# BiaPyX/BiaPy

Hardware: AMD Instinct MI355X
Metric: voxels/sec 3D ResUNet 128^3 patch (train: fwd+bwd+AdamW; sub-records: infer, sliding) (higher is better)
Workload: dtype f16 forward/activations + bf16 gradients (MFMA f16 / bf16, fp32 accumulate)

## Files before the change

biapy_amd/_lib.py:

```python
from __future__ import annotations

import ctypes as C
import os
from typing import Optional

import torch

_HERE = os.path.dirname(os.path.abspath(__file__))
LIB_PATH = os.environ.get("BPX_LIB_PATH") or os.path.join(_HERE, "libbiapy_amd.so")

F32, BF16, F16, U8, MIX16 = 0, 1, 2, 3, 4
ACT = {"none": 0, "linear": 0, "elu": 1, "relu": 2, "silu": 3, "leaky_relu": 4, "gelu": 5, "tanh": 6, "sigmoid": 7, "softplus": 8}
PK_K3, PK_K3_T, PK_K1, PK_DENSE, PK_DENSE_T, PK_CT, PK_CT_T, PK_CT4, PK_CT4_T = range(9)


class AxisGrid(C.Structure):
    _fields_ = [("n", C.c_int32), ("step", C.c_int32), ("last", C.c_int32), ("patch", C.c_int32), ("limit", C.c_int32)]


class Tensor(C.Structure):
    _fields_ = [("ptr", C.c_void_p), ("ld", C.c_int32), ("C", C.c_int32), ("cs", C.c_int64)]


NULL_T = Tensor(None, 0, 0, 0)
# ... 41 lines not shown
    "bpx_seg_loss_blocks": ([_i64], _i),
    "bpx_seg_loss_sums": ([_vp, _vp, _i64, _vp, _vp], _i),
    "bpx_seg_loss_bwd": ([_vp, _vp, _i64, _vp, _vp, _vp], _i),
    "bpx_seg_loss_finish": ([_vp, _i, _i64, _f, _f, _f, _vp, _vp, _vp], _i),
    "bpx_seg_loss_bwd_fused": ([_vp, _vp, _i64, _vp, _vp, _f, _f, _f, _vp, _vp], _i),
    "bpx_softmax_ce_blocks": ([_i64], _i),
    "bpx_softmax_ce_row": ([], _i),
    "bpx_softmax_ce_sums": ([_vp, _vp, _i, _i, _i64, _i, _vp, _vp, _vp], _i),
    "bpx_softmax_ce_finish": ([_vp, _i, _i64, _vp, _vp, _vp], _i),
    "bpx_softmax_ce_bwd": ([_vp, _vp, _i, _i, _i64, _i, _vp, _vp, _vp, _vp, _vp], _i),
    "bpx_dice_blocks": ([_i64], _i),
    "bpx_dice_row": ([], _i),
    "bpx_dice_sums": ([_vp, _vp, _i, _i, _i64, _i, _i, _vp, _i, _vp, _vp], _i),
    "bpx_dice_finish": ([_vp, _i, _i, _i64, _i, _i, C.c_double, C.c_double, C.c_double, _vp, _vp, _vp, _vp], _i),
    "bpx_dice_bwd": ([_vp, _vp, _i, _i, _i64, _i, _i, _i, _vp, _vp, _vp, _vp, _vp], _i),
    "bpx_chan_loss_finish": ([_vp, _i, _i, _i64, _vp, _vp, _vp], _i),
    "bpx_chan_loss_bwd_fused": ([_vp, _vp, _i, _i, _i64, C.c_uint, _vp, _vp, _vp, _vp], _i),
    "bpx_conv3d_fwd": ([_i, _i, _i, _i, _i, Tensor, _vp, _i, _vp, _vp, Tensor, _vp, _vp, Tensor, _vp, _vp], _i),
    "bpx_conv3d_fwd_pool": ([_i, _i, _i, _i, _i, Tensor, _vp, _i, _vp, _vp, Tensor, _vp, _vp, Tensor, _vp, _i, Tensor, _vp, _vp], _i),
    "bpx_conv3d_fwd_pool_supported": ([_i, _i, _i, _i, _i, _i, _i, _i], _i),
    "bpx_conv3d_fwd_shuffle": ([_i, _i, _i, _i, _i, Tensor, _vp, _i, _vp, _vp, _i, Tensor, _vp], _i),
    "bpx_conv3d_stats_tiles": ([_i, _i, _i, _i, _i, _i], _i),
    "bpx_conv3d_dgrad": ([_i, _i, _i, _i, _i, Tensor, _vp, Tensor, _vp, _i, Tensor, _vp, _vp], _i),
    "bpx_conv3d_wgrad": ([_i, _i, _i, _i, _i, Tensor, _vp, _i, Tensor, _i, _vp, _vp, _vp, _i64, _vp], _i),
    "bpx_conv3d_wgrad_db2": ([_i, _i, _i, _i, _i, Tensor, _vp, _i, Tensor, _i, _vp, _vp, _vp, _vp, _i64, _vp], _i),
    "bpx_conv3d_wgrad_workspace": ([_i, _i, _i, _i, _i, _i, _i], _i64),
    "bpx_conv3d_bwd_fused_supported": ([_i, _i, _i, _i, _i, _i, _i], _i),
    "bpx_conv3d_bwd_fused_stats_tiles": ([_i, _i, _i, _i, _i, _i], _i),
    "bpx_conv3d_bwd_fused_workspace": ([_i, _i, _i, _i, _i, _i], _i64),
    "bpx_conv3d_bwd_fused": ([_i, _i, _i, _i, _i, Tensor, _vp, Tensor, _vp, _i, Tensor, _vp, _vp, _vp, _vp, _vp, _i64, _vp], _i),
    "bpx_debug_set_bwd_fused": ([_i], _i),
    "bpx_debug_set_bwd_rs": ([_i], _i),
    "bpx_debug_set_conv_kg": ([_i], _i),
    "bpx_debug_set_tile_order": ([_i], _i),
    "bpx_debug_set_wgrad_cap": ([_i], _i),
    "bpx_debug_set_wgrad_k1": ([_i], _i),
    "bpx_debug_set_pw_stream": ([_i], _i),
    "bpx_debug_set_convt_k1": ([_i], _i),
    "bpx_debug_set_c1_persist": ([_i], _i),
    "bpx_convT3d_k2s2_wgrad_workspace": ([_i, _i, _i, _i, _i, _i, _i], _i64),
    "bpx_conv1x1_fwd": ([_i, _i, _i64, Tensor, _vp, _vp, Tensor, Tensor, _vp, Tensor, Tensor, _vp], _i),
    "bpx_conv1x1_fwd_split_wgrad_workspace": ([_i, _i, _i64, _i], _i64),
    "bpx_conv1x1_fwd_split_wgrad_query": ([_i, _i, _i64, Tensor, Tensor, Tensor, _vp, Tensor, Tensor], _i64),
    "bpx_conv1x1_fwd_split_wgrad": ([_i, _i, _i64, Tensor, _vp, Tensor, Tensor, _vp, Tensor, Tensor, _vp, _vp, _i64, _vp], _i),
    "bpx_conv1x1_fwd_split": ([_i, _i, _i64, Tensor, _vp, _vp, Tensor, Tensor, _vp, Tensor, Tensor, Tensor, _vp], _i),
    "bpx_convT3d_k2s2_fwd": ([_i, _i, _i, _i, _i, _i, Tensor, _vp, _vp, Tensor, _vp, _vp], _i),
    "bpx_convT3d_stats_tiles": ([_i, _i, _i, _i], _i),
    "bpx_convT3d_k2s2_dgrad": ([_i, _i, _i, _i, _i, _i, Tensor, _vp, Tensor, _vp], _i),
    "bpx_convT3d_k2s2_wgrad": ([_i, _i, _i, _i, _i, _i, Tensor, Tensor, _vp, _vp, _vp, _i64, _vp], _i),
    "bpx_convT3d_k2s2_bwd": ([_i, _i, _i, _i, _i, _i, Tensor, Tensor, _vp, Tensor, _vp, _vp, _vp, _i64, _vp], _i),
    "bpx_debug_set_convt_bwd": ([_i], _i),
    "bpx_debug_convt_bwd_launches": ([], _i),
    "bpx_norm_finalize": ([_vp, _i, _i, _i, _i64, _vp, _vp, _f, _i, _vp, _i, _i, _vp], _i),
    "bpx_norm_channel_sums": ([_vp, _i, _i, _i, _vp, _i, _i, _vp], _i),
    "bpx_groupnorm_finalize": ([_vp, _i, _i, _i64, _vp, _vp, _f, _i, _vp, _vp], _i),
    "bpx_groupnorm_bwd_finalize": ([_vp, _i, _i, _i64, _vp, _vp, _vp, _vp, _i, _vp, _vp], _i),
    "bpx_tensor_stats": ([_i, _i, _i64, Tensor, _vp, _vp], _i),
    "bpx_tensor_stats_tiles": ([_i64], _i),
    "bpx_norm_bwd_finalize": ([_vp, _i, _i, _i, _i64, _vp, _vp, _vp, _vp, _i, _vp, _vp], _i),
    "bpx_norm_bwd_finalize_deferred": ([_vp, _i, _i, _i, _i64, _vp, _vp, _vp, _vp, _i, _vp, _vp], _i),
    "bpx_batchnorm_finalize": ([_vp, _i, _i, _i, _i64, _vp, _vp, _f, _f, _vp, _vp, _vp, _vp, _i, _i, _vp], _i),
    "bpx_batchnorm_bwd_finalize": ([_vp, _i, _i, _i, _i64, _vp, _vp, _vp, _vp, _i, _vp, _vp], _i),
    "bpx_batchnorm_eval_records": ([_i, _vp, _i, _vp], _i),
    "bpx_gather3d_tables": ([_vp, _i, _i, _i, _i, _i, _vp, _i, _i, _i, _i, _vp, _vp], _i),
    "bpx_scatter3d_tables": ([_vp, _i, _vp, _i, _i, _i, _i, _vp, _i, _i, _i, _i, _vp], _i),
    "bpx_scatter3d_regions": ([_vp, _i, _i, _i, _i, _i, _vp, _vp, _i, _i, _i, _vp], _i),
# ... 202 lines not shown
```

biapy_amd/csrc/conv3d_igemm.hip:

```cpp
#include "conv3d_shared.h"

using namespace bpxconv;

namespace bpxconv { long long* g_conv_stamps = nullptr; }
#define g_stamps bpxconv::g_conv_stamps
extern "C" int bpx_debug_set_conv_stamps(void* p) { g_stamps = (long long*)p; return 0; }
static int g_use_ws = 0;
static int g_conv_kg = -1;
extern "C" int bpx_debug_set_conv_kg(int on) { g_conv_kg = on; return 0; }
static int64_t g_lean_min_vps = 32768;

namespace {

template <typename T, int EZ, int EY, int EX>
__device__ __forceinline__ void stage_block(unsigned char* smem, const T* __restrict__ src, int ld, int cs, int chunk, int n, int D, int H,
                                            int W, int oz, int oy, int ox, const bpx_norm_rec* __restrict__ norm, int C_norm,
                                            int act, int tid) {
  constexpr int KPL = ElemTraits<T>::KPL, GPT = 16 / KPL, VB = 16 * (int)sizeof(T);
  constexpr int PIECES = EZ * EY * EX * GPT;
  constexpr int UNR = 4;
  const int sub = tid % GPT;
  float sc[KPL], sh[KPL];
  if (norm) {
#pragma unroll
    for (int e = 0; e < KPL; ++e) {
      bpx_norm_rec r = norm[(size_t)n * C_norm + chunk * 16 + sub * KPL + e];
      sc[e] = r.scale; sh[e] = r.shift;
    }
  }
  const T* sbase = src + (size_t)chunk * cs + sub * KPL;
  for (int base = 0; base < PIECES; base += 256 * UNR) {
    u32x4_t buf[UNR];
    bool ok[UNR];
#pragma unroll
    for (int u = 0; u < UNR; ++u) {
      int idx = base + u * 256 + tid;
      ok[u] = false;
      buf[u] = u32x4_t{0u, 0u, 0u, 0u};
      if (idx < PIECES) {
        int hv = idx / GPT;
        int hx = hv % EX, hy = (hv / EX) % EY, hz = hv / (EX * EY);
        int gz = oz + hz, gy = oy + hy, gx = ox + hx;
// ... 1 lines not shown
          ok[u] = true;
          buf[u] = *reinterpret_cast<const u32x4_t*>(sbase + ((((size_t)n * D + gz) * H + gy) * W + gx) * (size_t)ld);
        }
      }
    }
#pragma unroll
    for (int u = 0; u < UNR; ++u) {
      int idx = base + u * 256 + tid;
      if (idx < PIECES) {
        u32x4_t v = buf[u];
        if (norm && ok[u]) {
          float f[KPL];
          unpack16<T>(v, f);
#pragma unroll
          for (int e = 0; e < KPL; ++e) f[e] = fmaf(sc[e], f[e], sh[e]);
          bpx_act_vec<std::is_same<T, float>::value, KPL>(f, act);
          v = pack16<T>(f);
        }
        *reinterpret_cast<u32x4_t*>(smem + (size_t)(idx / GPT) * VB + sub * 16) = v;
      }
    }
  }
}

__host__ __device__ constexpr int wreg_next(int s, int np, int per) {
  int k = 0;
  for (int t = np; t < s; ++t) {
    int c = t + 1 - k;
    k += c < per ? (c > 0 ? c : 0) : per;
  }
  return k;
}

template <typename T, int TZ, int TY, int TX, int NS, int EPI, int ACTK, typename TT = T, int KG = 1>
__global__ void __launch_bounds__(256 * KG, 2) conv3_kernel(const Conv3Params p) {
  using Tr = ElemTraits<T>;
  constexpr int KPL = Tr::KPL, GPT = 16 / KPL, VB = 16 * (int)sizeof(T);
  constexpr int HZ = TZ + 2, HY = TY + 2, HX = TX + 2, HV = HZ * HY * HX;
  constexpr int QTOT = 27 * GPT, STEPS = (QTOT + 3) / 4, QPAD = STEPS * 4;
  constexpr int MT = TZ * TY * TX / 16, MS = MT / 4;
  static_assert(MT % 4 == 0 && MS >= 1, "tile must give every wave at least one m-subtile");
  static_assert((HV * GPT + 255) / 256 <= STEPS, "one staged piece per MFMA step");
  static_assert(sizeof(T) != 2 || wreg_next(STEPS, (HV * GPT + 255) / 256, (STEPS + (STEPS - (HV * GPT + 255) / 256) - 1) / (STEPS - (HV * GPT + 255) / 256)) == STEPS, "weight re-load schedule must cover every fragment");
  constexpr int RED_BYTES = 4 * NS * 16 * 2 * 4;
  constexpr int BUFB = HV * VB;
  static_assert(NS * 16 * 2 * 4 * 4 <= RED_BYTES, "reduction scratch");
  constexpr int NBUF = 2;
  static_assert(KG == 1 || (TX == 8 && sizeof(T) == 2), "two K groups: the small-tile 16-bit instances only");
  constexpr int XCH_BYTES = KG == 2 ? MS * NS * 256 * 16 : 0;
  static_assert(XCH_BYTES <= KG * NBUF * BUFB, "accumulator exchange fits the halo buffers");
  __shared__ __attribute__((aligned(16))) unsigned char smem_all[KG * NBUF * BUFB + RED_BYTES];

  const int kg = KG == 2 ? __builtin_amdgcn_readfirstlane((int)(threadIdx.x >> 8)) : 0;
  unsigned char* const smem = smem_all + kg * NBUF * BUFB;
  const int tid = threadIdx.x & 255, lane = tid & 63, wave = tid >> 6;
  const int j = lane & 15, g = lane >> 4;
  const int tile = blockIdx.x % p.tilesPerSample, n = blockIdx.x / p.tilesPerSample;
  const int txi = tile % p.tilesX, tyi = (tile / p.tilesX) % p.tilesY, tzi = tile / (p.tilesX * p.tilesY);
  const int z0 = tzi * TZ, y0 = tyi * TY, x0 = txi * TX;
  const int co_base = blockIdx.y * 16 * NS;
  const int Cout = p.Cout;

  int stamp_i = 0;
#define BPX_STAMP() do { if (p.stamps && tid == 0 && kg == 0 && blockIdx.y == 0 && stamp_i < 15) p.stamps[(size_t)blockIdx.x * 16 + stamp_i++] = (long long)__builtin_readcyclecounter(); } while (0)
  BPX_STAMP();
  if (p.stamps && tid == 0 && kg == 0 && blockIdx.y == 0)
    p.stamps[(size_t)blockIdx.x * 16 + 15] =
        (long long)(((unsigned long long)__builtin_amdgcn_s_getreg((31 << 11) | 20) << 32) | (unsigned)__builtin_amdgcn_s_getreg((31 << 11) | 4));
  f32x4_t acc[MS][NS];
#pragma unroll
  for (int ms = 0; ms < MS; ++ms)
#pragma unroll
    for (int ns = 0; ns < NS; ++ns) acc[ms][ns] = f32x4_t{0.f, 0.f, 0.f, 0.f};

  static_assert(TZ == 4 && MS * 16 == TY * TX && (TX == 16 || TX == 8), "wave = z-slice mapping");
  constexpr int HSTR = (TX >= 16 ? 1 : 16 / TX) * HX * VB;
  constexpr int TSTR = 16 * VB;
  int hb0, tb0;
  {
    int t = (wave * MS) * 16 + j;
    int tz = t / (TY * TX), ty = (t / TX) % TY, tx = t % TX;
    hb0 = ((tz * HY + ty) * HX + tx) * VB;
    tb0 = t * VB;
  }
  const int cg_off = (GPT == 2 ? (g & 1) : g) * 16;
  const bool hi_tap = (GPT == 2) && (g >> 1);
  constexpr int NCLS = (GPT == 2) ? 4 : 1;
  int lbase[NCLS];
  if (GPT == 2) {
    lbase[0] = hb0 + cg_off + (hi_tap ? VB : 0);
    lbase[1 % NCLS] = hb0 + cg_off + (hi_tap ? HX * VB : 0);
    lbase[2 % NCLS] = hb0 + cg_off + (hi_tap ? HY * HX * VB : 0);
    lbase[NCLS - 1] = hb0 + cg_off;
  } else {
    lbase[0] = hb0 + cg_off;
  }

  constexpr int NPIECE = HV * GPT;
  constexpr int NP = (NPIECE + 255) / 256;
  const int sub = tid % GPT;
  uint32_t goff[NP];
#pragma unroll
  for (int u = 0; u < NP; ++u) {
    int idx = u * 256 + tid;
    goff[u] = 0xFFFFFFFFu;
    if (idx < NPIECE) {
      int hv = idx / GPT;
      int hx = hv % HX, hy = (hv / HX) % HY, hz = hv / (HX * HY);
      int gz = z0 - 1 + hz, gy = y0 - 1 + hy, gx = x0 - 1 + hx;
      if (gz >= 0 && gz < p.D && gy >= 0 && gy < p.H && gx >= 0 && gx < p.W)
        goff[u] = (uint32_t)((((uint32_t)gz * p.H + gy) * p.W + gx) * (uint32_t)p.x_ld);
    }
  }
  const T* __restrict__ xin = reinterpret_cast<const T*>(p.x) + (size_t)n * p.D * p.H * p.W * p.x_ld + sub * KPL;
  const T* __restrict__ wp = reinterpret_cast<const T*>(p.wp);
  const bpx_norm_rec* __restrict__ nrec = p.in_norm ? p.in_norm + (size_t)n * p.Cin + sub * KPL : nullptr;
  const int nchunks = p.Cin / 16;

  u32x4_t pbuf[NP];
  float psc[KPL], psh[KPL];

#define BPX_STAGE_PIECE(u, wbuf, next_chunk)                                                                  \
  do {                                                                                                        \
    const int idx_ = (u) * 256 + tid;                                                                         \
    if (idx_ < NPIECE) {                                                                                      \
      u32x4_t v_ = pbuf[u];                                                                                   \
      if (nrec && goff[u] != 0xFFFFFFFFu && !(p.dbg & 2)) {                                                   \
        float f_[KPL];                                                                                        \
        unpack16<T>(v_, f_);                                                                                  \
        if (ACTK == 1) { _Pragma("unroll") for (int e_ = 0; e_ < KPL; ++e_) f_[e_] = apply_act_rt<T, 1>(fmaf(psc[e_], f_[e_], psh[e_]), p.act); } \
        else { _Pragma("unroll") for (int e_ = 0; e_ < KPL; ++e_) f_[e_] = fmaf(psc[e_], f_[e_], psh[e_]);                    \
               bpx_act_vec<std::is_same<T, float>::value, KPL, ACTK == 2>(f_, p.act); }                                               \
        v_ = pack16<T>(f_);                                                                                   \
      }                                                                                                       \
      *reinterpret_cast<u32x4_t*>(smem + (wbuf) + (size_t)idx_ * 16) = v_;                                    \
      if ((next_chunk) < nchunks && goff[u] != 0xFFFFFFFFu && !(p.dbg & 4))                                   \
        pbuf[u] = *reinterpret_cast<const u32x4_t*>(xin + goff[u] + (size_t)(next_chunk) * p.x_cs);                       \
    }                                                                                                         \
  } while (0)
#define BPX_LOAD_NORM(chunk_)                                                                                 \
  do {                                                                                                        \
    if (nrec && (chunk_) < nchunks) {                                                                         \
      _Pragma("unroll") for (int e_ = 0; e_ < KPL; ++e_) {                                                    \
        bpx_norm_rec r_ = nrec[(chunk_) * 16 + e_];                                                           \
        psc[e_] = r_.scale; psh[e_] = r_.shift;                                                               \
      }                                                                                                       \
    }                                                                                                         \
  } while (0)

  BPX_STAMP();
  {
#pragma unroll
  for (int u = 0; u < NP; ++u) {
    pbuf[u] = u32x4_t{0u, 0u, 0u, 0u};
    if (goff[u] != 0xFFFFFFFFu) pbuf[u] = *reinterpret_cast<const u32x4_t*>(xin + goff[u] + (size_t)kg * p.x_cs);
  }
  BPX_LOAD_NORM(kg);
#pragma unroll
  for (int u = 0; u < NP; ++u) BPX_STAGE_PIECE(u, 0, kg + KG);
  BPX_LOAD_NORM(kg + KG);
  BPX_STAMP();
  __syncthreads();
  BPX_STAMP();

  constexpr bool WREG = (sizeof(T) == 2) && (STEPS * NS * 4 <= 112);
  constexpr int NWR = WREG ? STEPS : 1;
  constexpr int WSTEPS = STEPS - NP;
  constexpr int PER = WREG ? (STEPS + WSTEPS - 1) / WSTEPS : 1;
  u32x4_t wreg[NWR][NS];
  if (WREG) {
    const T* wl0 = wp + ((size_t)kg * QPAD * Cout + (size_t)g * Cout + co_base + j) * KPL;
#pragma unroll
    for (int s = 0; s < NWR; ++s)
#pragma unroll
      for (int ns = 0; ns < NS; ++ns) wreg[s][ns] = *reinterpret_cast<const u32x4_t*>(wl0 + ((size_t)s * 4 * Cout + ns * 16) * KPL);
  }
  constexpr bool SMALL = TX == 8;
  constexpr int WD = SMALL ? 3 : 1;
  constexpr int NAF = SMALL ? 2 : 1;
  u32x4_t wq[WREG ? 1 : WD + 1][NS];
  if (!WREG) {
    const T* wl0 = wp + ((size_t)kg * QPAD * Cout + (size_t)g * Cout + co_base + j) * KPL;
#pragma unroll
    for (int d = 0; d < WD; ++d)
#pragma unroll
      for (int ns = 0; ns < NS; ++ns) wq[d][ns] = *reinterpret_cast<const u32x4_t*>(wl0 + ((size_t)d * 4 * Cout + ns * 16) * KPL);
  }
  int cur = 0;
  for (int chunk = kg; chunk < nchunks; chunk += KG) {
    const int nxt = BUFB - cur;
    const bool stage_next = chunk + KG < nchunks;
    const T* wl = wp + ((size_t)chunk * QPAD * Cout + (size_t)g * Cout + co_base + j) * KPL;
    const T* wl1 = wl + (size_t)KG * QPAD * Cout * KPL;
    u32x4_t af[NAF][MS];
    auto read_frags = [&](int s_, u32x4_t* f) {
      const int tapA = (GPT == 2) ? bpx_tap_order_bf16(2 * s_) : s_;
      const int cls = (GPT == 2) ? (s_ < 9 ? 0 : s_ < 12 ? 1 : s_ == 12 ? 2 : 3) : 0;
      const int imm = tap_off<HY, HX, VB>(tapA);
#pragma unroll
      for (int ms = 0; ms < MS; ++ms) f[ms] = *reinterpret_cast<const u32x4_t*>(smem + lbase[cls] + ms * HSTR + imm);
    };
    if (NAF == 2) read_frags(0, af[0]);
#pragma unroll
    for (int s = 0; s < STEPS; ++s) {
      if (!WREG && s + WD < STEPS) {
#pragma unroll
        for (int ns = 0; ns < NS; ++ns)
          wq[WREG ? 0 : (s + WD) % (WD + 1)][ns] = *reinterpret_cast<const u32x4_t*>(wl + ((size_t)(s + WD) * 4 * Cout + ns * 16) * KPL);
      }
      if (NAF == 2) { if (s + 1 < STEPS) read_frags(s + 1, af[(s + 1) % NAF]); }
      else read_frags(s, af[0]);
      __builtin_amdgcn_sched_barrier(0);
#pragma unroll
      for (int ms = 0; ms < MS; ++ms) {
#pragma unroll
        for (int ns = 0; ns < NS; ++ns) acc[ms][ns] = mfma_step<T>(WREG ? wreg[WREG ? s : 0][ns] : wq[WREG ? 0 : s % (WD + 1)][ns], af[s % NAF][ms], acc[ms][ns]);
      }
      if (s < NP && stage_next) BPX_STAGE_PIECE(s < NP ? s : 0, nxt, chunk + 2 * KG);
      if (WREG && s >= NP && stage_next) {
        const int k0 = wreg_next(s, NP, PER), k1 = wreg_next(s + 1, NP, PER);
#pragma unroll
        for (int k = k0; k < k1; ++k) {
#pragma unroll
          for (int ns = 0; ns < NS; ++ns)
            wreg[WREG ? (k < STEPS ? k : 0) : 0][ns] = *reinterpret_cast<const u32x4_t*>(wl1 + ((size_t)k * 4 * Cout + ns * 16) * KPL);
        }
      }
    }
    if (!WREG && stage_next) {
#pragma unroll
      for (int d = 0; d < WD; ++d)
#pragma unroll
        for (int ns = 0; ns < NS; ++ns) wq[WREG ? 0 : d][ns] = *reinterpret_cast<const u32x4_t*>(wl1 + ((size_t)d * 4 * Cout + ns * 16) * KPL);
    }
    BPX_STAMP();
    BPX_LOAD_NORM(chunk + 2 * KG);
    const int flip = cur ? -BUFB : BUFB;
#pragma unroll
    for (int c = 0; c < NCLS; ++c) lbase[c] += flip;
    cur = nxt;
    __syncthreads();
    BPX_STAMP();
  }
  }
#undef BPX_STAGE_PIECE
#undef BPX_LOAD_NORM
  if constexpr (KG == 2) {
    f32x4_t* xch = reinterpret_cast<f32x4_t*>(smem_all);
    if (kg == 1) {
#pragma unroll
      for (int ms = 0; ms < MS; ++ms)
#pragma unroll
        for (int ns = 0; ns < NS; ++ns) xch[(ms * NS + ns) * 256 + tid] = acc[ms][ns];
    }
    __syncthreads();
    if (kg == 0) {
#pragma unroll
      for (int ms = 0; ms < MS; ++ms)
#pragma unroll
        for (int ns = 0; ns < NS; ++ns) acc[ms][ns] += xch[(ms * NS + ns) * 256 + tid];
    }
  }

  if (EPI == EPI_FWD && p.sc != nullptr && p.sc_C >= 16) {
    const T* __restrict__ scin = reinterpret_cast<const T*>(p.sc);
    const T* __restrict__ wsc = reinterpret_cast<const T*>(p.wsc);
    const int nch = p.sc_C / 16;
    for (int chunk = 0; chunk < nch; ++chunk) {
      __syncthreads();
      if (kg == 0) stage_block<T, TZ, TY, TX>(smem, scin, p.sc_ld, p.sc_cs, chunk, n, p.D, p.H, p.W, z0, y0, x0, nullptr, 0, 0, tid);
      __syncthreads();
      if (kg != 0) continue;
      const T* wl = wsc + ((size_t)chunk * 4 * Cout + (size_t)g * Cout + co_base + j) * KPL;
      u32x4_t wf[NS];
// ... 95 lines not shown
        if constexpr (std::is_same<T, float>::value) {
          *reinterpret_cast<f32x4_t*>(yp) = f32x4_t{v[0], v[1], v[2], v[3]};
        } else {
          *reinterpret_cast<u32x2_t*>(yp) = u32x2_t{pk16s<T>(v[0], v[1]), pk16s<T>(v[2], v[3])};
        }
      }
    }
  }

  }
  BPX_STAMP();
  if (p.part != nullptr) {
    float* red = reinterpret_cast<float*>(smem_all + KG * NBUF * BUFB);
#pragma unroll
    for (int ns = 0; ns < NS; ++ns)
#pragma unroll
      for (int r = 0; r < 4; ++r) {
        float a = s1[ns][r], b = s2[ns][r];
#pragma unroll
        for (int m = 1; m < 16; m <<= 1) { a += __shfl_xor(a, m, 64); b += __shfl_xor(b, m, 64); }
        if (j == 0 && kg == 0) {
          red[((wave * NS * 16) + ns * 16 + g * 4 + r) * 2 + 0] = a;
          red[((wave * NS * 16) + ns * 16 + g * 4 + r) * 2 + 1] = b;
        }
      }
    __syncthreads();
    if (tid < NS * 16 * 2 && kg == 0) {
      int c = tid >> 1, k = tid & 1;
      float a = red[(0 * NS * 16 + c) * 2 + k] + red[(1 * NS * 16 + c) * 2 + k] + red[(2 * NS * 16 + c) * 2 + k] +
                red[(3 * NS * 16 + c) * 2 + k];
      p.part[(((size_t)n * p.tilesPerSample + tile) * 2 + k) * Cout + co_base + c] = a;
    }
  }
}

template <typename T, int EPI, typename TT = T>
int launch_conv3(const Conv3Params& p0, const TileCfg& c, hipStream_t s) {
  Conv3Params p = p0;
  int tilesZ = cdiv(p.D, c.tz);
  p.tilesY = cdiv(p.H, c.ty);
  p.tilesX = cdiv(p.W, c.tx);
  p.tilesPerSample = tilesZ * p.tilesY * p.tilesX;
  { const char* e = getenv("BPX_CONV_DBG"); p.dbg = e ? atoi(e) : 0; }
  p.stamps = g_stamps;
  dim3 grid((unsigned)(p.N * p.tilesPerSample), (unsigned)(p.Cout / (16 * c.ns)));
  const bool elu = (EPI == EPI_FWD ? p.act : p.t_act) == BPX_ACT_ELU;
  const bool ext = (EPI == EPI_FWD ? p.act : p.t_act) > BPX_ACT_SILU;
  if constexpr (sizeof(T) == 2) {
    static const bool kg_env = getenv("BPX_CONV_KG") == nullptr || atoi(getenv("BPX_CONV_KG")) != 0;
    const int nchunks = p.Cin / 16;
    if ((g_conv_kg < 0 ? kg_env : g_conv_kg != 0) && c.tz == 4 && c.ty == 4 && c.tx == 8 && (c.ns == 2 || c.ns == 4) && nchunks >= 4 && nchunks % 2 == 0) {
#define LK(NS)                                                                                   \
      if (c.ns == NS) {                                                                          \
        if (elu) conv3_kernel<T, 4, 4, 8, NS, EPI, 1, TT, 2><<<grid, 512, 0, s>>>(p);            \
        else if (ext) conv3_kernel<T, 4, 4, 8, NS, EPI, 2, TT, 2><<<grid, 512, 0, s>>>(p);       \
        else conv3_kernel<T, 4, 4, 8, NS, EPI, 0, TT, 2><<<grid, 512, 0, s>>>(p);                \
        return 0;                                                                                \
      }
      LK(2) LK(4)
#undef LK
    }
  }
#define L(TZ, TY, TX, NS)                                                        \
  if (c.tz == TZ && c.ty == TY && c.tx == TX && c.ns == NS) {                    \
    if (elu) conv3_kernel<T, TZ, TY, TX, NS, EPI, 1, TT><<<grid, 256, 0, s>>>(p);    \
    else if (ext) conv3_kernel<T, TZ, TY, TX, NS, EPI, 2, TT><<<grid, 256, 0, s>>>(p);   \
    else conv3_kernel<T, TZ, TY, TX, NS, EPI, 0, TT><<<grid, 256, 0, s>>>(p);        \
    return 0;                                                                    \
  }
  if constexpr (sizeof(T) == 2) {
    L(4, 8, 16, 1)
  }
  L(4, 4, 16, 1) L(4, 4, 16, 2) L(4, 4, 16, 3) L(4, 4, 16, 4) L(4, 4, 8, 1) L(4, 4, 8, 2) L(4, 4, 8, 3) L(4, 4, 8, 4)
#undef L
  return 1;
}

}

extern "C" int bpx_debug_set_conv_ws(int on) {
  if (on == 10 || on == 11) { g_lean_min_vps = on == 10 ? 262144 : 32768; return 0; }
  g_use_ws = on;
  return 0;
}

static bool use_lean(int dtype, const Conv3Params& p) {
  const int64_t vps = (int64_t)p.D * p.H * p.W, vox = vps * p.N;
  if ((dtype != BPX_BF16 && dtype != BPX_F16) || !(g_use_ws == 5 || (g_use_ws == 0 && vps >= g_lean_min_vps))) return false;
  if ((p.in_norm && p.act > BPX_ACT_SILU) || (p.t_norm && p.t_act > BPX_ACT_SILU)) return false;
  const int64_t ldmax = std::max<int64_t>(std::max(p.x_ld, p.y_ld), std::max(p.sc ? p.sc_ld : 0, p.t ? p.t_ld : 0));
  auto al = [](const void* q) { return ((uintptr_t)q & 15) == 0; };
  auto ext = [](int cs, int C) { return cs == 16 ? (int64_t)0 : (int64_t)cs * (C / 16); };
  const int64_t planar = std::max(std::max(ext(p.x_cs, p.Cin), ext(p.y_cs, p.Cout)), std::max(p.sc ? ext(p.sc_cs, p.sc_C) : 0, p.t ? ext(p.t_cs, p.Cout) : 0));
  return p.W > 8 && vox * ldmax < (1ll << 31) && planar < (1ll << 31) && vox < (1ll << 30) && al(p.bias) && al(p.bias_sc) && al(p.wsc) && al(p.in_norm) && al(p.t_norm);
}

extern "C" int bpx_conv3d_stats_tiles(int dtype, int N, int D, int H, int W, int Cout) {
  TileCfg c = pick_cfg(dtype, D, H, W, Cout);
  int t = cdiv(D, c.tz) * cdiv(H, c.ty) * cdiv(W, c.tx);
  (void)N;
  return t;
}

static int check_tensor(const char* fn, const char* name, const bpx_tensor& t, int esize, bool need16) {
  BPX_CHECK(t.ptr != nullptr, "%s: %s.ptr is null", fn, name);
  BPX_CHECK(t.C >= 1 && t.ld >= (t.cs ? 16 : t.C), "%s: %s has ld %d < C %d", fn, name, t.ld, t.C);
  if (need16) {
    BPX_CHECK(t.C % 16 == 0, "%s: %s.C = %d must be a multiple of 16", fn, name, t.C);
    BPX_CHECK(((uintptr_t)t.ptr % 16) == 0 && ((size_t)t.ld * esize) % 16 == 0, "%s: %s must be 16-byte aligned (ptr and ld)", fn, name);
  }
  return 0;
}

static int check_planar(const char* fn, const char* name, const bpx_tensor& t, int N, int D, int H, int W) {
  if (t.ptr == nullptr || t.cs == 0) return 0;
  const int64_t vox = (int64_t)N * D * H * W;
  BPX_CHECK(t.ld >= 16 && t.cs % 8 == 0 && t.cs >= (vox - 1) * t.ld + 16 && t.cs < (1ll << 31), "%s: %s has chunk stride %lld for %lld voxels of pitch %d", fn,
            name, (long long)t.cs, (long long)vox, t.ld);
  return 0;
}

static int conv3d_fwd_impl(const char* fn, int dtype, int N, int D, int H, int W, bpx_tensor x, const bpx_norm_rec* in_norm_d, int act,
                           const void* w_packed_d, const float* bias_d, bpx_tensor sc, const void* w_sc_d,
                           const float* bias_sc_d, bpx_tensor y, float* stats_part_d, int pool_sz, bpx_tensor pooled,
                           float* pool_stats_part_d, bpx_stream_t stream) {
  BPX_CHECK(dtype == BPX_BF16 || dtype == BPX_F32 || dtype == BPX_F16, "%s: dtype must be BF16, F16 (forward only) or F32", fn);
  int es = (int)dtype_size(dtype);
  BPX_CHECK(N > 0 && D > 0 && H > 0 && W > 0, "%s: empty volume", fn);
  if (check_tensor(fn, "x", x, es, true) || check_tensor(fn, "y", y, es, true)) return 1;
  BPX_CHECK(w_packed_d != nullptr, "%s: packed weights are null", fn);
  if (sc.ptr) {
    BPX_CHECK(w_sc_d != nullptr, "%s: shortcut weights are null", fn);
    if (sc.C != 1 && check_tensor(fn, "sc", sc, es, true)) return 1;
  }
// ... 114 lines not shown
```

include/biapy_amd.h:

```cpp
#ifndef BIAPY_AMD_H
#define BIAPY_AMD_H

#include <stdint.h>

#ifdef __cplusplus
extern "C" {
#endif

typedef void* bpx_stream_t;

enum bpx_dtype { BPX_F32 = 0, BPX_BF16 = 1, BPX_F16 = 2, BPX_U8 = 3,
                 BPX_MIX16 = 4 };
enum bpx_act { BPX_ACT_NONE = 0, BPX_ACT_ELU = 1, BPX_ACT_RELU = 2, BPX_ACT_SILU = 3, BPX_ACT_LEAKY_RELU = 4, BPX_ACT_GELU = 5, BPX_ACT_TANH = 6,
               BPX_ACT_SIGMOID = 7, BPX_ACT_SOFTPLUS = 8, BPX_ACT_LAST = 8 };
enum bpx_pad_mode { BPX_PAD_REFLECT = 0, BPX_PAD_ZEROS = 1 };

int bpx_version(void);
const char* bpx_last_error(void);
int bpx_selftest_layouts(float* out_d , bpx_stream_t stream);
int bpx_debug_set_wgrad_tr(int use_tr);
int bpx_debug_set_conv_stamps(void* stamps_d);
int bpx_debug_set_conv_ws(int on);
int bpx_debug_set_conv_occ(int wg_per_cu);
int bpx_debug_set_conv_zm(int mode);
// ... 69 lines not shown
                      double eps, double weight_decay, int decoupled, const float* gscale_d, bpx_stream_t stream);

int bpx_conv3d_fwd(int dtype, int N, int D, int H, int W, bpx_tensor x, const bpx_norm_rec* in_norm_d, int act,
                   const void* w_packed_d, const float* bias_d, bpx_tensor sc, const void* w_sc_packed_d,
                   const float* bias_sc_d, bpx_tensor y, float* stats_part_d, bpx_stream_t stream);
int bpx_conv3d_stats_tiles(int dtype, int N, int D, int H, int W, int Cout);
int bpx_conv3d_fwd_pool(int dtype, int N, int D, int H, int W, bpx_tensor x, const bpx_norm_rec* in_norm_d, int act,
                        const void* w_packed_d, const float* bias_d, bpx_tensor sc, const void* w_sc_packed_d,
                        const float* bias_sc_d, bpx_tensor y, float* stats_part_d, int pool_sz, bpx_tensor pooled,
                        float* pool_stats_part_d, bpx_stream_t stream);
int bpx_conv3d_fwd_pool_supported(int dtype, int N, int D, int H, int W, int x_ld, int y_ld, int Cout);
int bpx_conv3d_fwd_shuffle(int dtype, int N, int D, int H, int W, bpx_tensor x, const bpx_norm_rec* in_norm_d, int act, const void* w_packed_d,
                           const float* bias_d, int s, bpx_tensor y, bpx_stream_t stream);

int bpx_conv3d_dgrad(int dtype, int N, int D, int H, int W, bpx_tensor dy, const void* w_packed_T_d,
                     bpx_tensor t, const bpx_norm_rec* t_norm_d, int act, bpx_tensor g,
                     float* red_part_d, bpx_stream_t stream);

int64_t bpx_conv3d_wgrad_workspace(int N, int D, int H, int W, int Cin, int Cout, int k);
int bpx_conv3d_wgrad(int dtype, int N, int D, int H, int W, bpx_tensor x, const bpx_norm_rec* in_norm_d, int act,
                     bpx_tensor dy, int k, float* dw_d, float* db_d, void* ws_d, int64_t ws_bytes, bpx_stream_t stream);
int bpx_conv3d_wgrad_db2(int dtype, int N, int D, int H, int W, bpx_tensor x, const bpx_norm_rec* in_norm_d, int act,
                         bpx_tensor dy, int k, float* dw_d, float* db_d, float* db2_d, void* ws_d, int64_t ws_bytes, bpx_stream_t stream);

int bpx_conv3d_bwd_fused_supported(int dtype, int N, int D, int H, int W, int Ct, int Cdy);
int bpx_conv3d_bwd_fused_stats_tiles(int N, int D, int H, int W, int Ct, int Cdy);
int64_t bpx_conv3d_bwd_fused_workspace(int N, int D, int H, int W, int Ct, int Cdy);
int bpx_conv3d_bwd_fused(int dtype, int N, int D, int H, int W, bpx_tensor dy, const void* w_packed_T_d, bpx_tensor t,
                         const bpx_norm_rec* t_norm_d, int act, bpx_tensor g, float* red_part_d, float* dw_d, float* db_d, float* db2_d,
                         void* ws_d, int64_t ws_bytes, bpx_stream_t stream);
int bpx_debug_set_bwd_fused(int bits);
int bpx_debug_set_bwd_rs(int mask);
int bpx_debug_set_conv_kg(int on);

int bpx_wgrad_defer_begin(void);
int bpx_wgrad_defer_flush(bpx_stream_t stream);

typedef struct bpx_nbwd_coef { float a, b, c0, pad; } bpx_nbwd_coef;

int bpx_conv1x1_fwd(int dtype, int N, int64_t voxels, bpx_tensor x, const void* w_packed_d, const float* bias_d,
                    bpx_tensor g, bpx_tensor t, const bpx_nbwd_coef* coef_d, bpx_tensor addend, bpx_tensor y,
                    bpx_stream_t stream);
int bpx_conv1x1_fwd_split(int dtype, int N, int64_t voxels, bpx_tensor x, const void* w_packed_d, const float* bias_d,
                          bpx_tensor g, bpx_tensor t, const bpx_nbwd_coef* coef_d, bpx_tensor addend, bpx_tensor y_lo,
                          bpx_tensor y_hi, bpx_stream_t stream);
int64_t bpx_conv1x1_fwd_split_wgrad_workspace(int dtype, int N, int64_t voxels, int K);
int64_t bpx_conv1x1_fwd_split_wgrad_query(int dtype, int N, int64_t voxels, bpx_tensor x, bpx_tensor g, bpx_tensor t, const void* coef_d,
                                          bpx_tensor y_lo, bpx_tensor y_hi);
int bpx_conv1x1_fwd_split_wgrad(int dtype, int N, int64_t voxels, bpx_tensor x, const void* w_packed_d, bpx_tensor g, bpx_tensor t,
                                const bpx_nbwd_coef* coef_d, bpx_tensor y_lo, bpx_tensor y_hi, float* dw_d, void* ws_d, int64_t ws_bytes,
                                bpx_stream_t stream);

int bpx_convT3d_k2s2_fwd(int dtype, int N, int D, int H, int W, int sz, bpx_tensor x, const void* w_packed_d,
                         const float* bias_d, bpx_tensor y, float* stats_part_d, bpx_stream_t stream);
int bpx_convT3d_stats_tiles(int D, int H, int W, int sz);
int bpx_convT3d_k2s2_dgrad(int dtype, int N, int D, int H, int W, int sz, bpx_tensor dy, const void* w_packed_T_d,
                           bpx_tensor dx, bpx_stream_t stream);
int64_t bpx_convT3d_k2s2_wgrad_workspace(int N, int D, int H, int W, int sz, int Cin, int Cout);
int bpx_convT3d_k2s2_wgrad(int dtype, int N, int D, int H, int W, int sz, bpx_tensor x, bpx_tensor dy,
                           float* dw_d , float* db_d ,
                           void* ws_d, int64_t ws_bytes, bpx_stream_t stream);
int bpx_convT3d_k2s2_bwd(int dtype, int N, int D, int H, int W, int sz, bpx_tensor x, bpx_tensor dy, const void* w_packed_T_d,
                         bpx_tensor dx, float* dw_d, float* db_d, void* ws_d, int64_t ws_bytes, bpx_stream_t stream);
int bpx_debug_set_convt_bwd(int on);
int bpx_debug_convt_bwd_launches(void);

// ... 154 lines not shown
```

Baseline: 1.066 billion.

## Stage conv3d weight fragments into LDS via buffer_load-to-LDS double buffering

```diff
diff --git a/biapy_amd/_lib.py b/biapy_amd/_lib.py
--- a/biapy_amd/_lib.py
+++ b/biapy_amd/_lib.py
@@ -97,6 +97,9 @@
     "bpx_debug_set_bwd_fused": ([_i], _i),
     "bpx_debug_set_bwd_rs": ([_i], _i),
     "bpx_debug_set_conv_kg": ([_i], _i),
+    "bpx_debug_set_conv_wlds": ([_i], _i),
+    "bpx_conv3d_wlds_used": ([_i, _i, _i, _i, _i, _i, _i], _i),
+    "bpx_conv3d_wlds_lds_bytes": ([_i, _i, _i], _i),
     "bpx_debug_set_tile_order": ([_i], _i),
     "bpx_debug_set_wgrad_cap": ([_i], _i),
     "bpx_debug_set_wgrad_k1": ([_i], _i),
diff --git a/biapy_amd/csrc/conv3d_igemm.hip b/biapy_amd/csrc/conv3d_igemm.hip
--- a/biapy_amd/csrc/conv3d_igemm.hip
+++ b/biapy_amd/csrc/conv3d_igemm.hip
@@ -8,6 +8,8 @@
 static int g_use_ws = 0;
 static int g_conv_kg = -1;
 extern "C" int bpx_debug_set_conv_kg(int on) { g_conv_kg = on; return 0; }
+static int g_conv_wlds = -1;
+extern "C" int bpx_debug_set_conv_wlds(int on) { g_conv_wlds = on; return 0; }
 static int64_t g_lean_min_vps = 32768;
 
 namespace {
@@ -75,7 +77,16 @@
   return k;
 }
 
-template <typename T, int TZ, int TY, int TX, int NS, int EPI, int ACTK, typename TT = T, int KG = 1>
+__device__ __forceinline__ void wdma16(const u32x4_t& rsrc, uint32_t lds, uint32_t voff) {
+  asm volatile("s_mov_b32 m0, %0\n\ts_nop 0\n\tbuffer_load_dwordx4 %1, %2, 0 offen lds" : : "s"(lds), "v"(voff), "s"(rsrc) : "memory", "m0");
+}
+
+__host__ __device__ constexpr int wlds_parts(int ns, int kg) { return (kg == 2 && ns == 4) ? 2 : 1; }
+__host__ __device__ constexpr int wlds_lds_bytes(int ns, int kg, int wl) {
+  return kg * 2 * (6 * 6 * 10 * 32) + 4 * ns * 16 * 2 * 4 + (wl ? kg * 2 * (14 / wl) * ns * 1024 : 0);
+}
+
+template <typename T, int TZ, int TY, int TX, int NS, int EPI, int ACTK, typename TT = T, int KG = 1, int WL = 0>
 __global__ void __launch_bounds__(256 * KG, 2) conv3_kernel(const Conv3Params p) {
   using Tr = ElemTraits<T>;
   constexpr int KPL = Tr::KPL, GPT = 16 / KPL, VB = 16 * (int)sizeof(T);
@@ -92,7 +103,11 @@
   static_assert(KG == 1 || (TX == 8 && sizeof(T) == 2), "two K groups: the small-tile 16-bit instances only");
   constexpr int XCH_BYTES = KG == 2 ? MS * NS * 256 * 16 : 0;
   static_assert(XCH_BYTES <= KG * NBUF * BUFB, "accumulator exchange fits the halo buffers");
-  __shared__ __attribute__((aligned(16))) unsigned char smem_all[KG * NBUF * BUFB + RED_BYTES];
+  static_assert(WL == 0 || (TX == 8 && sizeof(T) == 2 && STEPS % WL == 0), "weights in LDS: the small-tile 16-bit instances only");
+  constexpr int WPS = WL ? STEPS / WL : STEPS;
+  constexpr int WPART = WL ? WPS * NS * 1024 : 0;
+  static_assert(WL == 0 || (KG * NBUF * BUFB + RED_BYTES + KG * 2 * WPART == wlds_lds_bytes(NS, KG, WL) && wlds_lds_bytes(NS, KG, WL) <= 160 * 1024), "LDS plan");
+  __shared__ __attribute__((aligned(16))) unsigned char smem_all[KG * NBUF * BUFB + RED_BYTES + KG * 2 * WPART];
 
   const int kg = KG == 2 ? __builtin_amdgcn_readfirstlane((int)(threadIdx.x >> 8)) : 0;
   unsigned char* const smem = smem_all + kg * NBUF * BUFB;
@@ -159,6 +174,33 @@
   const T* __restrict__ wp = reinterpret_cast<const T*>(p.wp);
   const bpx_norm_rec* __restrict__ nrec = p.in_norm ? p.in_norm + (size_t)n * p.Cin + sub * KPL : nullptr;
   const int nchunks = p.Cin / 16;
+
+  typedef __attribute__((address_space(3))) void* lds_ptr_t;
+  unsigned char* const wsm = smem_all + KG * NBUF * BUFB + RED_BYTES + kg * 2 * WPART;
+  u32x4_t rs_w = u32x4_t{0u, 0u, 0u, 0u};
+  uint32_t wlds = 0u, wvoff = 0u;
+  int wave_s = 0;
+  if constexpr (WL > 0) {
+    const uint64_t a = reinterpret_cast<uint64_t>(p.wp);
+    rs_w = u32x4_t{(uint32_t)__builtin_amdgcn_readfirstlane((int)(uint32_t)a), (uint32_t)__builtin_amdgcn_readfirstlane((int)(uint32_t)(a >> 32)) & 0xFFFFu,
+                   (uint32_t)nchunks * (uint32_t)(QPAD * 16) * (uint32_t)Cout, 0x00020000u};
+    wlds = (uint32_t)__builtin_amdgcn_readfirstlane((int)(uint32_t)(uintptr_t)(lds_ptr_t)wsm);
+    wvoff = (uint32_t)((g * Cout + co_base + j) * 16);
+    wave_s = __builtin_amdgcn_readfirstlane(wave);
+  }
+  auto issue_w = [&](int chunk_, int s0, uint32_t dst) {
+    const uint32_t src = wvoff + (uint32_t)(chunk_ * QPAD + s0 * 4) * (uint32_t)Cout * 16u;
+#pragma unroll
+    for (int i = 0; i < (WPS * NS + 3) / 4; ++i) {
+      const int q = i * 4 + wave_s;
+      if (q < WPS * NS) wdma16(rs_w, dst + (uint32_t)q * 1024u, src + (uint32_t)(q / NS) * (uint32_t)Cout * 64u + (uint32_t)(q % NS) * 256u);
+    }
+  };
+  if constexpr (WL > 0) {
+    issue_w(kg, 0, wlds);
+    if (WL == 2) issue_w(kg, WPS, wlds + WPART);
+    else if (kg + KG < nchunks) issue_w(kg + KG, 0, wlds + WPART);
+  }
 
   u32x4_t pbuf[NP];
   float psc[KPL], psh[KPL];
@@ -203,10 +245,11 @@
   for (int u = 0; u < NP; ++u) BPX_STAGE_PIECE(u, 0, kg + KG);
   BPX_LOAD_NORM(kg + KG);
   BPX_STAMP();
+  if constexpr (WL > 0) __builtin_amdgcn_s_waitcnt(0x0F70);
   __syncthreads();
   BPX_STAMP();
 
-  constexpr bool WREG = (sizeof(T) == 2) && (STEPS * NS * 4 <= 112);
+  constexpr bool WREG = WL == 0 && (sizeof(T) == 2) && (STEPS * NS * 4 <= 112);
   constexpr int NWR = WREG ? STEPS : 1;
   constexpr int WSTEPS = STEPS - NP;
   constexpr int PER = WREG ? (STEPS + WSTEPS - 1) / WSTEPS : 1;
@@ -222,7 +265,7 @@
   constexpr int WD = SMALL ? 3 : 1;
   constexpr int NAF = SMALL ? 2 : 1;
   u32x4_t wq[WREG ? 1 : WD + 1][NS];
-  if (!WREG) {
+  if (!WREG && WL == 0) {
     const T* wl0 = wp + ((size_t)kg * QPAD * Cout + (size_t)g * Cout + co_base + j) * KPL;
 #pragma unroll
     for (int d = 0; d < WD; ++d)
@@ -230,6 +273,8 @@
       for (int ns = 0; ns < NS; ++ns) wq[d][ns] = *reinterpret_cast<const u32x4_t*>(wl0 + ((size_t)d * 4 * Cout + ns * 16) * KPL);
   }
   int cur = 0;
+  int wrd = lane * 16;
+  uint32_t wcur = 0u;
   for (int chunk = kg; chunk < nchunks; chunk += KG) {
     const int nxt = BUFB - cur;
     const bool stage_next = chunk + KG < nchunks;
@@ -243,21 +288,35 @@
 #pragma unroll
       for (int ms = 0; ms < MS; ++ms) f[ms] = *reinterpret_cast<const u32x4_t*>(smem + lbase[cls] + ms * HSTR + imm);
     };
+    u32x4_t wf[WL ? 2 : 1][NS];
+    if constexpr (WL > 0) {
+#pragma unroll
+      for (int u = 0; u < NP; ++u)
+#pragma unroll
+        for (int e = 0; e < 4; ++e) { uint32_t v_ = pbuf[u][e]; asm volatile("" : "+v"(v_)); pbuf[u][e] = v_; }
+    }
+    auto read_w = [&](int s_, u32x4_t* f) {
+#pragma unroll
+      for (int ns = 0; ns < NS; ++ns)
+        f[ns] = *reinterpret_cast<const u32x4_t*>(wsm + wrd + (WL == 2 ? (s_ / WPS) * WPART : 0) + ((s_ % WPS) * NS + ns) * 1024);
+    };
     if (NAF == 2) read_frags(0, af[0]);
+    if constexpr (WL > 0) read_w(0, wf[0]);
 #pragma unroll
     for (int s = 0; s < STEPS; ++s) {
-      if (!WREG && s + WD < STEPS) {
+      if (!WREG && WL == 0 && s + WD < STEPS) {
 #pragma unroll
         for (int ns = 0; ns < NS; ++ns)
           wq[WREG ? 0 : (s + WD) % (WD + 1)][ns] = *reinterpret_cast<const u32x4_t*>(wl + ((size_t)(s + WD) * 4 * Cout + ns * 16) * KPL);
       }
       if (NAF == 2) { if (s + 1 < STEPS) read_frags(s + 1, af[(s + 1) % NAF]); }
       else read_frags(s, af[0]);
+      if constexpr (WL > 0) { if (s + 1 < STEPS && (s + 1) % WPS != 0) read_w(s + 1, wf[WL ? (s + 1) % 2 : 0]); }
       __builtin_amdgcn_sched_barrier(0);
 #pragma unroll
       for (int ms = 0; ms < MS; ++ms) {
 #pragma unroll
-        for (int ns = 0; ns < NS; ++ns) acc[ms][ns] = mfma_step<T>(WREG ? wreg[WREG ? s : 0][ns] : wq[WREG ? 0 : s % (WD + 1)][ns], af[s % NAF][ms], acc[ms][ns]);
+        for (int ns = 0; ns < NS; ++ns) acc[ms][ns] = mfma_step<T>(WL ? wf[WL ? s % 2 : 0][ns] : WREG ? wreg[WREG ? s : 0][ns] : wq[WREG ? 0 : s % (WD + 1)][ns], af[s % NAF][ms], acc[ms][ns]);
       }
       if (s < NP && stage_next) BPX_STAGE_PIECE(s < NP ? s : 0, nxt, chunk + 2 * KG);
       if (WREG && s >= NP && stage_next) {
@@ -269,8 +328,16 @@
             wreg[WREG ? (k < STEPS ? k : 0) : 0][ns] = *reinterpret_cast<const u32x4_t*>(wl1 + ((size_t)k * 4 * Cout + ns * 16) * KPL);
         }
       }
-    }
-    if (!WREG && stage_next) {
+      if constexpr (WL == 2) {
+        if (s + 1 == WPS) {
+          __builtin_amdgcn_s_waitcnt(0x0F70);
+          __syncthreads();
+          if (stage_next) issue_w(chunk + KG, 0, wlds);
+          read_w(s + 1, wf[(s + 1) % 2]);
+        }
+      }
+    }
+    if (!WREG && WL == 0 && stage_next) {
 #pragma unroll
       for (int d = 0; d < WD; ++d)
 #pragma unroll
@@ -282,7 +349,14 @@
 #pragma unroll
     for (int c = 0; c < NCLS; ++c) lbase[c] += flip;
     cur = nxt;
+    if constexpr (WL > 0) __builtin_amdgcn_s_waitcnt(0x0F70);
     __syncthreads();
+    if constexpr (WL == 1) {
+      if (chunk + 2 * KG < nchunks) issue_w(chunk + 2 * KG, 0, wlds + wcur);
+      wrd += wcur ? -WPART : WPART;
+      wcur = (uint32_t)WPART - wcur;
+    }
+    if constexpr (WL == 2) { if (stage_next) issue_w(chunk + KG, WPS, wlds + WPART); }
     BPX_STAMP();
   }
   }
@@ -444,6 +518,36 @@
       p.part[(((size_t)n * p.tilesPerSample + tile) * 2 + k) * Cout + co_base + c] = a;
     }
   }
+}
+
+struct SmallForm { int kg, wl; };
+static int wlds_mode() {
+  static const int env = getenv("BPX_CONV_WLDS") == nullptr ? -1 : (atoi(getenv("BPX_CONV_WLDS")) != 0 ? 1 : 0);
+  return g_conv_wlds < 0 ? env : (g_conv_wlds != 0 ? 1 : 0);
+}
+static int device_cus() {
+  static int n = 0;
+  if (n == 0) {
+    int dev = 0;
+    if (hipGetDevice(&dev) != hipSuccess || hipDeviceGetAttribute(&n, hipDeviceAttributeMultiprocessorCount, dev) != hipSuccess || n <= 0) n = 256;
+  }
+  return n;
+}
+static SmallForm small_form(const TileCfg& c, int es, int N, int D, int H, int W, int Cin, int Cout, int mode, int cus) {
+  SmallForm f{1, 0};
+  if (es != 2 || c.tz != 4 || c.ty != 4 || c.tx != 8) return f;
+  static const bool kg_env = getenv("BPX_CONV_KG") == nullptr || atoi(getenv("BPX_CONV_KG")) != 0;
+  const int nchunks = Cin / 16;
+  if ((g_conv_kg < 0 ? kg_env : g_conv_kg != 0) && (c.ns == 2 || c.ns == 4) && nchunks >= 4 && nchunks % 2 == 0) f.kg = 2;
+  if (mode == 0 || (int64_t)nchunks * 56 * 16 * Cout >= (1ll << 31)) return f;
+  const int wl = wlds_parts(c.ns, f.kg);
+  if (mode < 0) {
+    const int64_t wgs = (int64_t)N * cdiv(D, 4) * cdiv(H, 4) * cdiv(W, 8) * (Cout / (16 * c.ns));
+    if (nchunks / f.kg < 4) return f;
+    if (wlds_lds_bytes(c.ns, f.kg, wl) > 80 * 1024 && wgs > 3 * (int64_t)cus) return f;
+  }
+  f.wl = wl;
+  return f;
 }
 
 template <typename T, int EPI, typename TT = T>
@@ -459,19 +563,17 @@
   const bool elu = (EPI == EPI_FWD ? p.act : p.t_act) == BPX_ACT_ELU;
   const bool ext = (EPI == EPI_FWD ? p.act : p.t_act) > BPX_ACT_SILU;
   if constexpr (sizeof(T) == 2) {
-    static const bool kg_env = getenv("BPX_CONV_KG") == nullptr || atoi(getenv("BPX_CONV_KG")) != 0;
-    const int nchunks = p.Cin / 16;
-    if ((g_conv_kg < 0 ? kg_env : g_conv_kg != 0) && c.tz == 4 && c.ty == 4 && c.tx == 8 && (c.ns == 2 || c.ns == 4) && nchunks >= 4 && nchunks % 2 == 0) {
-#define LK(NS)                                                                                   \
-      if (c.ns == NS) {                                                                          \
-        if (elu) conv3_kernel<T, 4, 4, 8, NS, EPI, 1, TT, 2><<<grid, 512, 0, s>>>(p);            \
-        else if (ext) conv3_kernel<T, 4, 4, 8, NS, EPI, 2, TT, 2><<<grid, 512, 0, s>>>(p);       \
-        else conv3_kernel<T, 4, 4, 8, NS, EPI, 0, TT, 2><<<grid, 512, 0, s>>>(p);                \
-        return 0;                                                                                \
-      }
-      LK(2) LK(4)
+    const SmallForm f = small_form(c, 2, p.N, p.D, p.H, p.W, p.Cin, p.Cout, wlds_mode(), wlds_mode() < 0 ? device_cus() : 0);
+#define LK(NS, KG, WL)                                                                                        \
+    if (c.ns == NS && f.kg == KG && f.wl == WL) {                                                             \
+      if (elu) conv3_kernel<T, 4, 4, 8, NS, EPI, 1, TT, KG, WL><<<grid, 256 * KG, 0, s>>>(p);                  \
+      else if (ext) conv3_kernel<T, 4, 4, 8, NS, EPI, 2, TT, KG, WL><<<grid, 256 * KG, 0, s>>>(p);             \
+      else conv3_kernel<T, 4, 4, 8, NS, EPI, 0, TT, KG, WL><<<grid, 256 * KG, 0, s>>>(p);                      \
+      return 0;                                                                                               \
+    }
+    LK(2, 2, 0) LK(4, 2, 0)
+    LK(1, 1, 1) LK(2, 1, 1) LK(3, 1, 1) LK(4, 1, 1) LK(2, 2, 1) LK(4, 2, 2)
 #undef LK
-    }
   }
 #define L(TZ, TY, TX, NS)                                                        \
   if (c.tz == TZ && c.ty == TY && c.tx == TX && c.ns == NS) {                    \
@@ -512,6 +614,18 @@
   int t = cdiv(D, c.tz) * cdiv(H, c.ty) * cdiv(W, c.tx);
   (void)N;
   return t;
+}
+
+extern "C" int bpx_conv3d_wlds_used(int dtype, int N, int D, int H, int W, int Cin, int Cout) {
+  if (dtype != BPX_BF16 && dtype != BPX_F16 && dtype != BPX_MIX16) return 0;
+  if (N <= 0 || D <= 0 || H <= 0 || W <= 0 || Cin < 16 || Cin % 16 != 0 || Cout < 16 || Cout % 16 != 0) return 0;
+  const TileCfg c = pick_cfg(BPX_BF16, D, H, W, Cout);
+  const int mode = wlds_mode();
+  return small_form(c, 2, N, D, H, W, Cin, Cout, mode, mode < 0 ? device_cus() : 0).wl != 0 ? 1 : 0;
+}
+extern "C" int bpx_conv3d_wlds_lds_bytes(int ns, int kg, int staged) {
+  if (ns < 1 || ns > 4 || kg < 1 || kg > 2 || (kg == 2 && ns != 2 && ns != 4)) return -1;
+  return wlds_lds_bytes(ns, kg, staged ? wlds_parts(ns, kg) : 0);
 }
 
 static int check_tensor(const char* fn, const char* name, const bpx_tensor& t, int esize, bool need16) {
diff --git a/include/biapy_amd.h b/include/biapy_amd.h
--- a/include/biapy_amd.h
+++ b/include/biapy_amd.h
@@ -125,6 +125,9 @@
 int bpx_debug_set_bwd_fused(int bits);
 int bpx_debug_set_bwd_rs(int mask);
 int bpx_debug_set_conv_kg(int on);
+int bpx_debug_set_conv_wlds(int on);
+int bpx_conv3d_wlds_used(int dtype, int N, int D, int H, int W, int Cin, int Cout);
+int bpx_conv3d_wlds_lds_bytes(int ns, int kg, int staged);
 
 int bpx_wgrad_defer_begin(void);
 int bpx_wgrad_defer_flush(bpx_stream_t stream);
```

Result: no change. 1.075 billion (median of 6 runs) (+0.8%).
